# wedevxer/CUDA-AcceleratedVectorDatabaseEngine

Hardware: AMD Instinct MI355X
Metric: QPS + p99 latency, 10M×768D IVF-Flat k=10 nprobe=32, 1/2/4/8 MI355X (higher is better)
Workload: dtype fp32; 1 GPU; 10M x 768D IVF-Flat L2, nlist 4096, nprobe 32, batch 64, k 10; nvec=10000000, dim=768, nlist=4096, nprobe=32, batch=64, k=10, train_vectors=100000, parallelism=single GPU; 3 batches in flight

## Files before the change

cuda-acceleratedvectordatabaseengine_amd/csrc/engine.cpp:

```cpp
#include "engine.hpp"

#include <cmath>

#include "remove.hpp"
#include "remove_plan.hpp"

namespace vdbe {
thread_local std::string g_last_error;

namespace group {
void train_device(vdb_ivf* g, const float* d_v, uint64_t n);
void set_centroids(vdb_ivf* g, const float* c);
void add_host(vdb_ivf* g, const float* v, const uint64_t* ids, const uint32_t* lists, uint64_t n);
void add_device(vdb_ivf* g, const float* d_v, const uint64_t* d_ids, const uint32_t* d_lists, uint64_t n);
uint64_t gpu_bytes(const vdb_ivf* g, bool allocated);
void set_option(vdb_ivf* g, const std::string& name, int64_t value);
void synchronize(vdb_ivf* g);
uint64_t remove_ids(vdb_ivf* g, const std::vector<uint64_t>& sorted);
}

inline void no_group(const vdb_ivf* h, const char* what) {
    require(!h->is_group(), std::string(what) + " is not available on a group handle", VDB_ERR_UNSUPPORTED);
}
}

extern "C" {

const char* vdb_last_error(void) { return g_last_error.c_str(); }
const char* vdb_version(void) { return "vdb_ivf 0.1.0 (gfx950)"; }
#ifndef VDB_BUILD_ID
#define VDB_BUILD_ID "unknown"
#endif
const char* vdb_build_id(void) { return VDB_BUILD_ID; }

int vdb_device_count(int* count) {
    return guarded([&] {
        require(count != nullptr, "null count");
        HIPCHECK(hipGetDeviceCount(count));
    });
}

int vdb_ivf_create(const vdb_ivf_config* cfg, vdb_ivf** out) {
    return guarded([&] {
        require(cfg && out, "null argument");
        require(cfg->dimension > 0 && cfg->nlist > 0, "Invalid configuration: dimension and nlist must be > 0");
        require(cfg->metric >= 0 && cfg->metric <= 2, "unknown metric");
        require(cfg->nlist < (1u << 19) - 1, "nlist above 524286 is not supported", VDB_ERR_UNSUPPORTED);
        auto* h = new vdb_ivf();
        try {
            h->dim = cfg->dimension;
            h->nlist = cfg->nlist;
            h->d4 = (cfg->dimension + 4 * vdbk::kTileAlign - 1) / (4 * vdbk::kTileAlign) * vdbk::kTileAlign;
            h->dp = h->d4 * 4;
            h->metric = cfg->metric;
            h->device = cfg->device;
            h->max_gpu_memory = cfg->max_gpu_memory == ~0ull ? 0 : cfg->max_gpu_memory;
            h->set_device();
            HIPCHECK(hipStreamCreateWithFlags(&h->stream, hipStreamNonBlocking));
            for (auto& sl : h->slots) {
                HIPCHECK(hipStreamCreateWithFlags(&sl.side, hipStreamNonBlocking));
                HIPCHECK(hipEventCreateWithFlags(&sl.fork, hipEventDisableTiming));
                HIPCHECK(hipEventCreateWithFlags(&sl.join, hipEventDisableTiming));
                HIPCHECK(hipEventCreateWithFlags(&sl.done, hipEventDisableTiming));
            }
            h->cent_rm.ensure((size_t)h->nlist * h->dp);
            h->cent_il.ensure(cdiv(h->nlist, 64) * h->d4 * 64);
            HIPCHECK(hipMemsetAsync(h->cent_rm.p, 0, (size_t)h->nlist * h->dp * 4, h->stream));
            h->refresh_centroid_layout();
            h->count.assign(h->nlist, 0);
            h->owned.assign(h->nlist, 1);
            h->block_off.assign(h->nlist, 0);
            h->upload_directory();
        } catch (...) {
            delete h;
            throw;
        }
        *out = h;
    });
}

int vdb_ivf_destroy(vdb_ivf* h) {
    return guarded([&] {
        if (!h) return;
        (void)hipSetDevice(h->device);
        (void)hipStreamSynchronize(h->stream);
        delete h;
// ... 905 lines not shown
```

cuda-acceleratedvectordatabaseengine_amd/csrc/kernels.hpp:

```cpp
#pragma once
#include <hip/hip_runtime.h>
#include <stdint.h>

namespace vdbk {

constexpr int kMaxSegBlocks = 16;
constexpr int kTilePipe = 16;
constexpr uint32_t kMfmaBlockedRows = 1024;
#ifndef VDB_MERGE_BLOCKS
#define VDB_MERGE_BLOCKS 1024
#endif
constexpr uint32_t kMergeBlocks = VDB_MERGE_BLOCKS;
#ifndef VDB_TILE_PIPE_NARROW
#define VDB_TILE_PIPE_NARROW 4
#endif
constexpr int kTilePipeNarrow = VDB_TILE_PIPE_NARROW;
#ifndef VDB_SCAN_DIAG
#define VDB_SCAN_DIAG 0
#endif
constexpr int kTileAlign = kTilePipe;
constexpr int kMergeFan = 32;
constexpr int kWideGroup = 16;
constexpr int kWaveQueries = 16;
constexpr int kWideMinSeg = 4;
// ... 33 lines not shown
void launch_coarse_mfma(int metric, const float* cent_rm, uint32_t nlist, uint32_t dp, const float* qpad,
                        uint32_t B, float* approx, float* delta, hipStream_t s);
uint32_t rerank_rows(uint32_t dp, int regs);
void launch_select_rerank(int metric, int regs, const float* approx, const float* delta, const float* cent_rm,
                          uint32_t nlist, uint32_t dp, const float* qpad, uint32_t B, uint32_t P, uint32_t* cand,
                          uint32_t* probes, hipStream_t s);
void launch_assign_rerank(int metric, const float* approx, const float* delta, const float* cent_rm,
                          uint32_t nlist, uint32_t dp, const float* rows, uint32_t n, uint32_t* out, hipStream_t s);
void launch_select(int regs, const float* cd, uint32_t nlist, uint32_t B, uint32_t P, uint32_t* probes,
                   hipStream_t s);
void launch_plan(const uint32_t* probes, const uint32_t* nseg_local, const uint32_t* count_local,
                 uint32_t B, uint32_t P, uint32_t group, int wide, uint32_t segs_item, ScanItem* items, ScanItem* items_w,
                 uint32_t* counters, uint32_t* sorted_pair, uint32_t* part_base_sorted, uint32_t* part_base_qp,
                 uint32_t* nseg_qp, uint32_t* l1base_qp, uint2* l1_items, unsigned long long* stats,
                 uint32_t* thr, uint32_t mfma_min, hipStream_t s);
void launch_merge_partials(int regs, uint32_t grid_items, const uint32_t* probes, const uint32_t* count_global,
                           const uint32_t* nseg_qp, const uint32_t* part_base_qp, const uint32_t* l1base_qp,
                           const uint2* l1_items, const uint32_t* counters, const float* part_d,
                           const uint64_t* part_i, uint32_t k, float* l1_d, uint64_t* l1_i, hipStream_t s);
struct ScanArgs {
    const float4* __restrict__ arena;
    const uint64_t* __restrict__ ids;
    const uint64_t* __restrict__ block_off;
    const uint32_t* __restrict__ count;
    const float* __restrict__ qpad;
    const ScanItem* __restrict__ items;
    const ScanItem* __restrict__ items_w;
    const uint32_t* __restrict__ counters;
    const uint32_t* __restrict__ sorted_pair;
    const uint32_t* __restrict__ part_base_sorted;
    float* __restrict__ part_d;
    uint64_t* __restrict__ part_i;
    uint32_t d4;
    uint32_t k;
    uint32_t wide_stride;
    uint32_t* work;
    uint32_t seg_blocks;
    uint32_t segs_item;
    uint32_t fused;
    uint32_t* thr;
    uint32_t mfma_min;
    unsigned long long* mstats;
    const uint4* __restrict__ shadow = nullptr;
    const float* __restrict__ rows = nullptr;
    const float4* __restrict__ meta = nullptr;
    const uint16_t* __restrict__ qres = nullptr;
    const float4* __restrict__ pst = nullptr;
    const float* __restrict__ sscale = nullptr;
    const float* __restrict__ qscale = nullptr;
    uint32_t dp = 0;
    uint32_t P = 0;
    uint32_t wide_q = 16;
    uint32_t thr_every = 1;
    uint32_t* thr4 = nullptr;
    uint4* cand = nullptr;
    uint32_t cand_cap = 0;
    uint32_t* ccount = nullptr;
    uint32_t* ovf = nullptr;
    uint4* floor_out = nullptr;
    uint32_t floor_seq = 0;
    float* ublist = nullptr;
    uint32_t* ubcnt = nullptr;
    uint32_t rows_layout = 0;
    unsigned long long* stamps = nullptr;
    uint32_t stamps_cap = 0;
    uint32_t stamp_batch = 0;
};
size_t scan_wide_lds(uint32_t d4, uint32_t k, int waves);
bool scan_wide_fits(uint32_t d4, uint32_t k, int waves);
void launch_scan_narrow(int metric, int regs, uint32_t grid_blocks, const ScanArgs& a, hipStream_t s);
void launch_scan_wide(int metric, uint32_t grid_blocks, const ScanArgs& a, hipStream_t s, int waves = 4);
size_t scan_bounded_lds(uint32_t d4, uint32_t k);
bool scan_bounded_fits(uint32_t d4, uint32_t k);
void launch_scan_bounded(int metric, uint32_t grid_blocks, const ScanArgs& a, hipStream_t s);
bool scan_screen_fits(uint32_t k, uint32_t dp, uint32_t wq, bool deferred);
size_t screen_exact_lds(uint32_t d4);
void launch_gather_cache_rows(const float4* cache, uint32_t d4, const ulonglong2* src, uint32_t n, float* rows,
                              hipStream_t s);
size_t screen_shadow_u4(uint64_t blocks, uint32_t d4, bool i8 = false);
void launch_screen_build(const float4* arena, uint64_t blocks, uint32_t d4, const uint32_t* block_list,
                         const float* cent_rm, uint4* shadow, float* rows, float4* meta, hipStream_t s, float* sscale = nullptr);
void launch_screen_pairs(int metric, const float* q, uint32_t B, uint32_t P, const uint32_t* probes,
                         const float* cent_rm, uint32_t dp, uint16_t* qres, float4* pst, uint32_t* thr4, hipStream_t s,
                         uint32_t* scnt = nullptr, uint32_t* ovf = nullptr, uint32_t* counters = nullptr,
                         uint32_t* ubcnt = nullptr, float* qscale = nullptr);
void launch_scan_screen(int metric, uint32_t grid_blocks, const ScanArgs& a, hipStream_t s);
void launch_screen_collect(int metric, uint32_t grid_blocks, const ScanArgs& a, hipStream_t s);
void launch_screen_select(const ScanArgs& a, uint32_t BP, uint32_t* scnt, uint32_t* soff, uint2* surv,
                          const uint32_t* ovf, hipStream_t s, float* slb = nullptr);
void launch_screen_recheck(int metric, const ScanArgs& a, uint32_t BP, const uint32_t* probes, uint32_t* nseg_qp,
                           const uint32_t* soff, const uint32_t* scnt, const uint2* surv, const uint32_t* ovf,
                           const float* fetched, float* sdist, uint32_t max_surv, uint32_t smax, hipStream_t s,
                           const float* slb = nullptr);
void launch_tier_recheck(int phase, int metric, const ScanArgs& a, uint32_t BP, uint32_t* nseg_qp, const uint32_t* soff,
                         const uint32_t* scnt, const uint2* surv, const float* slb, uint8_t* mark, const uint32_t* rowmap,
                         const float* fetched, float* sdist, hipStream_t s);
void launch_slot_merge(int regs, const uint32_t* probes, const uint32_t* count_global,
                       const uint32_t* nseg_qp, const uint32_t* part_base_qp, const uint32_t* l1base_qp,
                       const float* part_d, const uint64_t* part_i, const float* l1_d, const uint64_t* l1_i,
                       uint32_t BP, uint32_t k, float* slot_d, uint64_t* slot_i, hipStream_t s);
void launch_query_merge(int regs, const uint32_t* probes, const uint32_t* count_global, const float* slot_d,
                        const uint64_t* slot_i, const float* carry_d, const uint64_t* carry_i,
                        uint32_t B, uint32_t P, uint32_t k, int stale, const uint32_t* req_start, uint32_t b0,
                        float* out_d, uint64_t* out_i, hipStream_t s);
void launch_carry(const uint32_t* probes, const uint32_t* count_global, uint32_t B, uint32_t P, uint32_t k,
                  const float* slot_d, const uint64_t* slot_i, const uint32_t* req_start, uint32_t b0,
                  float* carry_d, uint64_t* carry_i, hipStream_t s);
void launch_merge_fused(int regs, const uint32_t* probes, const uint32_t* count_global, const uint32_t* nseg_qp,
                        const uint32_t* part_base_qp, const float* part_d, const uint64_t* part_i, uint32_t B,
                        uint32_t P, uint32_t k, int stale, const uint32_t* req_start, uint32_t b0, const float* carry_d,
                        const uint64_t* carry_i, float* slot_d, uint64_t* slot_i, float* carry_nd, uint64_t* carry_ni,
                        float* out_d, uint64_t* out_i, hipStream_t s);
void launch_rank_merge(int regs, const float* d, const uint64_t* i, uint64_t d_stride, uint64_t i_stride,
                       uint32_t nranks, uint32_t n, uint32_t k, float* out_d, uint64_t* out_i, hipStream_t s);
void launch_fill_empty(uint64_t n, float* d, uint64_t* i, hipStream_t s);

void launch_interleave(const float* rows, uint64_t n, uint32_t dp, float4* blocks, hipStream_t s);
void launch_scatter_rows(const float* rows, const uint64_t* row_ids, const uint32_t* order, uint64_t n,
                         uint32_t dp, const uint64_t* dest_slot, float4* arena, uint64_t* arena_ids,
                         hipStream_t s);
void launch_copy_lists(const float4* old_arena, const uint64_t* old_ids, const uint64_t* old_off,
                       const uint64_t* new_off, const uint32_t* nblocks, uint32_t nlist, uint32_t d4,
                       float4* new_arena, uint64_t* new_ids, hipStream_t s);
void launch_export_list(const float4* arena, const uint64_t* ids, uint64_t block_off, uint32_t count,
                        uint32_t dim, uint32_t d4, float* out, uint64_t* out_ids, hipStream_t s);
void launch_assign(int metric, const float* vpad, uint64_t n, uint32_t dp, const float4* cent_il,
                   uint32_t nlist, uint32_t* out, hipStream_t s);
void launch_histogram(const uint32_t* keys, uint64_t n, uint32_t* counts, hipStream_t s);
void launch_mindist_init(float* mind, uint64_t n, hipStream_t s);
void launch_mindist_update(const float4* v_il, uint64_t n, uint32_t d4, const float* centroid_row,
                           float* mind, hipStream_t s);
void launch_centroid_update(const float* vpad, uint32_t dp, const uint32_t* order, const uint32_t* offsets,
                            const uint32_t* counts, uint32_t nlist, uint32_t dim, float* cent_rm,
                            hipStream_t s);
void launch_iota(uint32_t* out, uint64_t n, hipStream_t s);
void launch_slots_from_order(const uint32_t* sorted_keys, uint64_t n, const uint64_t* group_start,
                             const uint64_t* list_base_slot, uint64_t* dest_slot, hipStream_t s);
void launch_gen_normal(float* out, uint64_t n, uint64_t seed, uint64_t offset, hipStream_t s);
void launch_gen_mixture(float* out, uint64_t rows, uint32_t dim, const float* centers, uint32_t ncomp, float sigma,
                        uint64_t seed, uint64_t row0, hipStream_t s);
// ... 7 lines not shown
```

cuda-acceleratedvectordatabaseengine_amd/csrc/screen.hip:

```cpp
#pragma clang fp contract(off)

#include <hip/hip_runtime.h>

#include <algorithm>
#include <stdexcept>
#include <cfloat>
#include <type_traits>

#include "kernels.hpp"
#include "scan_common.hpp"
#include "wave_topk.hpp"

namespace vdbk {

typedef __bf16 bf16x8 __attribute__((ext_vector_type(8)));
typedef float f32x4 __attribute__((ext_vector_type(4)));
typedef uint32_t u32x4 __attribute__((ext_vector_type(4)));
typedef int i32x4 __attribute__((ext_vector_type(4)));

constexpr float kScreenHuge = 1125899906842624.0f;
constexpr int kRing = 512;
#ifndef VDB_SCREEN_EXACT_PIPE
#define VDB_SCREEN_EXACT_PIPE 4
#endif
constexpr int kExactPipe = VDB_SCREEN_EXACT_PIPE;
#ifndef VDB_SCREEN_EXACT_PIPE_END
#define VDB_SCREEN_EXACT_PIPE_END 8
#endif
constexpr int kExactPipeEnd = VDB_SCREEN_EXACT_PIPE_END;
#ifndef VDB_SCREEN_DIAG
#define VDB_SCREEN_DIAG 0
#endif

__device__ __forceinline__ uint32_t bf16_bits(float f) {
    const uint32_t b = __float_as_uint(f);
    const uint32_t ex = b & 0x7F800000u;
    if (ex == 0) return 0u;
    if (ex == 0x7F800000u) return 0x7FC0u;
    return (b + 0x7FFFu + ((b >> 16) & 1u)) >> 16;
}
__device__ __forceinline__ float bf16_val(uint32_t h) { return __uint_as_float(h << 16); }

__device__ __forceinline__ uint4 pack_bf16x8(const float4 lo, const float4 hi) {
    uint4 r;
    r.x = bf16_bits(lo.x) | (bf16_bits(lo.y) << 16);
    r.y = bf16_bits(lo.z) | (bf16_bits(lo.w) << 16);
    r.z = bf16_bits(hi.x) | (bf16_bits(hi.y) << 16);
    r.w = bf16_bits(hi.z) | (bf16_bits(hi.w) << 16);
    return r;
}

__device__ __forceinline__ float4 resid(const float4 x, const float4 c) {
    return make_float4((float)((double)x.x - c.x), (float)((double)x.y - c.y), (float)((double)x.z - c.z),
                       (float)((double)x.w - c.w));
}

__device__ __forceinline__ float ru(double v) { return __double2float_ru(v * (1.0 + 0x1p-30)); }
// ... 594 lines not shown
        if ((wv & 1) == 0 && (wv == 0 || split)) screen_partials(a, it, q0, nqh, seg0, it_d + ko, it_i + ko, true);
    }
    if (a.fused) drain_narrow();
}


__device__ __forceinline__ void block_sort64(float (&u)[4]) {
    const int l = lane_id() & 15;
    bitonic64_step<2, 1>(u, l);
    bitonic64_step<4, 2>(u, l), bitonic64_step<4, 1>(u, l);
    bitonic64_step<8, 4>(u, l), bitonic64_step<8, 2>(u, l), bitonic64_step<8, 1>(u, l);
    bitonic64_step<16, 8>(u, l), bitonic64_step<16, 4>(u, l), bitonic64_step<16, 2>(u, l), bitonic64_step<16, 1>(u, l);
    bitonic64_step<32, 16>(u, l), bitonic64_step<32, 8>(u, l), bitonic64_step<32, 4>(u, l);
    bitonic64_step<32, 2>(u, l), bitonic64_step<32, 1>(u, l);
    bitonic64_step<64, 32>(u, l), bitonic64_step<64, 16>(u, l), bitonic64_step<64, 8>(u, l);
    bitonic64_step<64, 4>(u, l), bitonic64_step<64, 2>(u, l), bitonic64_step<64, 1>(u, l);
}
__device__ __forceinline__ void merge_sorted64(float (&rl)[4], const float (&u)[4]) {
    const int l = lane_id() & 15;
#pragma unroll
    for (int v = 0; v < 4; ++v) {
        const float rv = __uint_as_float((uint32_t)__builtin_amdgcn_mov_dpp((int)__float_as_uint(u[3 - v]), 0x140, 0xF,
                                                                            0xF, false));
        rl[v] = fminf(rl[v], rv);
    }
    bitonic64_step<64, 32>(rl, l), bitonic64_step<64, 16>(rl, l), bitonic64_step<64, 8>(rl, l);
    bitonic64_step<64, 4>(rl, l), bitonic64_step<64, 2>(rl, l), bitonic64_step<64, 1>(rl, l);
}
__device__ __forceinline__ float row_elem(const float (&u)[4], int e) {
    const int v = e & 3;
    const float x = v == 0 ? u[0] : v == 1 ? u[1] : v == 2 ? u[2] : u[3];
    return __shfl(x, (lane_id() & ~15) + (e >> 2));
}

struct CandChunk {
    uint32_t base = 0, left = 0;
    uint32_t next = 0;
    uint32_t real = 0;
    bool pending = false;
};
__device__ __forceinline__ void pad_cand(const ScanArgs& a, uint32_t base, uint32_t n) {
    for (uint32_t i = (uint32_t)lane_id(); i < n; i += 64)
        if (base + i < a.cand_cap) a.cand[base + i] = make_uint4(~0u, 0u, 0u, ~0u);
}
__device__ __forceinline__ void finish_cand(const ScanArgs& a, CandChunk& cc) {
    pad_cand(a, cc.base, cc.left);
    if (cc.pending) pad_cand(a, cc.next, kCandChunk);
    if (cc.real && lane_id() == 0) atomicAdd(a.ccount + (kCtrReal - kCtrCand), cc.real);
    cc.left = 0;
    cc.real = 0;
    cc.pending = false;
}

template <int M, int KD, int NG, bool I8, bool W2>
__device__ __forceinline__ void collect_segment(const ScanArgs& a, const ScanItem it, const int q0, const int nq,
                                                const uint32_t seg, float4* rl_lds, uint32_t* s_thr,
                                                const float4* s_pst, const float* s_qsc, float4* s_mt, float* s_vs,
                                                const uint32_t residue, CandChunk& cc) {
    const int lane = lane_id();
    const uint32_t dp = a.dp, ks = dp >> (I8 ? 6 : 5);
    const uint32_t count = a.count[it.list];
    const uint32_t seg_vectors = a.seg_blocks * 64;
    const uint64_t b0 = a.block_off[it.list] + (uint64_t)seg * a.seg_blocks;
    const uint32_t v0 = seg * seg_vectors;
    const uint32_t nv = min(count - v0, seg_vectors);
    const uint32_t nb = (nv + 63) >> 6;
    const int k = (int)a.k, kq = ((int)a.k + 3) / 4;
    const uint32_t* pairs = a.sorted_pair + it.pair_start + q0;
    const float cm = (float)(4 * dp + 16) * 0x1.02p-24f;
    const float cr = (float)(dp + 2) * 0x1.02p-24f;
    const float cu = 0x1.02p-23f;
    auto pair_of = [&](int g) -> uint32_t {
        const uint32_t pr = pairs[g];
        return (pr >> 16) * a.P + (pr & 0xFFFFu);
    };
    const uint4* qa_row[NG];
#pragma unroll
    for (int gg = 0; gg < NG; ++gg)
        qa_row[gg] = (const uint4*)((const char*)a.qres + (size_t)pair_of(min(16 * gg + (lane & 15), nq - 1)) * dp *
                                                              (I8 ? 1 : 2)) +
                     (lane >> 4);
    uint32_t collected = 0;
    float gthr[NG][4], gq4[NG][4];
#pragma unroll
    for (int gg = 0; gg < NG; ++gg)
#pragma unroll
        for (int r = 0; r < 4; ++r) gthr[gg][r] = gq4[gg][r] = __builtin_inff();
    const uint32_t thr_every = W2 ? a.thr_every : 1u;
    const uint32_t spl = it.pair_start + q0 + min(lane & (16 * NG - 1), nq - 1);

    const uint4* sp = a.shadow + b0 * (uint64_t)ks * 256 + lane;
    uint4 xa[KD][4], qa[NG][KD];
#pragma unroll
    for (int u = 0; u < KD; ++u) {
#pragma unroll
        for (int vt = 0; vt < 4; ++vt) xa[u][vt] = ld_nt_u4(sp + (size_t)(u * 4 + vt) * 64);
#pragma unroll
        for (int gg = 0; gg < NG; ++gg) qa[gg][u] = qa_row[gg][4 * (u % ks)];
    }
    using AccT = std::conditional_t<I8, i32x4, f32x4>;
    for (uint32_t j = 0; j < nb; ++j) {
        const uint64_t mslot = (b0 + j) * 64 + lane;
        const float4 mt_l = a.meta[mslot];
        float vs_l = 0.0f;
        if constexpr (I8) vs_l = a.sscale[mslot];
        const bool thr_now = j % thr_every == 0;
        uint32_t gt_l = 0u;
        uint4 t4_l = make_uint4(0u, 0u, 0u, 0u);
        if (thr_now) {
            gt_l = a.thr[spl];
            t4_l = *(const uint4*)(a.thr4 + (size_t)spl * 4);
        }
        const bool reserve = !cc.pending && cc.left < kCandChunk / 2;
        uint32_t reply = 0;
        if (reserve && lane == 0) reply = atomicAdd(a.ccount, kCandChunk);
        AccT acc[NG][4];
#pragma unroll
        for (int gg = 0; gg < NG; ++gg)
#pragma unroll
            for (int vt = 0; vt < 4; ++vt) acc[gg][vt] = AccT{0, 0, 0, 0};
        for (uint32_t s0 = 0; s0 < ks; s0 += KD) {
            static_for<0, KD>([&](auto uu) {
                constexpr int u = decltype(uu)::value;
#pragma unroll
                for (int gg = 0; gg < NG; ++gg) {
                    if constexpr (I8) {
                        const i32x4 A = as_i32x4(qa[gg][u]);
#pragma unroll
                        for (int vt = 0; vt < 4; ++vt)
                            acc[gg][vt] =
                                __builtin_amdgcn_mfma_i32_16x16x64_i8(A, as_i32x4(xa[u][vt]), acc[gg][vt], 0, 0, 0);
                    } else {
                        const bf16x8 A = as_bf16x8(qa[gg][u]);
#pragma unroll
                        for (int vt = 0; vt < 4; ++vt)
                            acc[gg][vt] =
                                __builtin_amdgcn_mfma_f32_16x16x32_bf16(A, as_bf16x8(xa[u][vt]), acc[gg][vt], 0, 0, 0);
                    }
                }
                const uint64_t nxt = (uint64_t)j * ks + s0 + u + KD;
#pragma unroll
                for (int vt = 0; vt < 4; ++vt) xa[u][vt] = ld_nt_u4(sp + (nxt * 4 + vt) * 64);
#pragma unroll
                for (int gg = 0; gg < NG; ++gg) qa[gg][u] = qa_row[gg][4 * ((s0 + u + KD) % ks)];
            });
        }
        s_mt[lane] = mt_l;
        if constexpr (I8) s_vs[lane] = vs_l;
        if (reserve) {
            cc.next = __builtin_amdgcn_readfirstlane(reply);
            cc.pending = true;
        }
        float gthr_l = 0.0f, gq4_l = 0.0f;
        if (thr_now) {
            const float th4 =
                fmaxf(fmaxf(ord_dec(t4_l.x), ord_dec(t4_l.y)), fmaxf(ord_dec(t4_l.z), ord_dec(t4_l.w)));
            gthr_l = fminf(ord_dec(gt_l), th4);
            gq4_l = ord_dec(residue == 0 ? t4_l.x : residue == 1 ? t4_l.y : residue == 2 ? t4_l.z : t4_l.w);
        }
        __builtin_amdgcn_fence(__ATOMIC_RELEASE, "wavefront");
#pragma unroll
        for (int gg = 0; gg < NG; ++gg) {
            const int g0 = 16 * gg;
            float ubv[4][4];
            float4 pst[4];
            float qsc[4];
#pragma unroll
            for (int r = 0; r < 4; ++r) {
                const int gc = min(g0 + 4 * (lane >> 4) + r, nq - 1);
                pst[r] = s_pst[gc];
                if constexpr (I8) qsc[r] = s_qsc[gc];
            }
#pragma unroll
            for (int vt = 0; vt < 4; ++vt) {
                const float4 mt = s_mt[16 * vt + (lane & 15)];
                float vsc = 0.0f;
                if constexpr (I8) vsc = s_vs[16 * vt + (lane & 15)];
                const bool valid = j * 64 + 16 * vt + (lane & 15) < nv;
#pragma unroll
                for (int r = 0; r < 4; ++r) {
                    float dot;
                    if constexpr (I8) dot = (float)acc[gg][vt][r] * (qsc[r] * vsc);
                    else dot = acc[gg][vt][r];
                    const float4 ps = pst[r];
                    const float approx = M == kL2 ? (ps.x + mt.x) - 2.0f * dot : -(ps.x + dot);
                    const float an = ps.y + ps.z, bn = mt.y + mt.z;
                    const float cs = an * mt.z + ps.z * bn + ps.z * mt.z;
                    float del;
                    if (M == kL2) {
                        const float rest = 2.0f * (cs + cm * (an * bn)) + cu * (ps.x + mt.x + fabsf(approx));
                        del = rest + cr * (fabsf(approx) + rest);
                    } else {
                        del = cs + cm * (an * bn) + cr * (ps.y * mt.w) + cu * (ps.y * ps.w + an * bn + fabsf(approx));
                    }
                    del = del * 1.001f + 1e-30f;
                    const float ub = approx + del;
                    if constexpr (I8) acc[gg][vt][r] = __float_as_int(approx - del);
// ... 119 lines not shown
    }
    if (a.mstats && lane == 0) {
        atomicAdd(&a.mstats[0], (unsigned long long)collected);
        atomicAdd(&a.mstats[1], (unsigned long long)nb);
    }
}

__device__ __forceinline__ void overflow_item(const ScanArgs& a, uint32_t pair_start, uint32_t npairs, uint32_t t0,
                                              uint32_t nt) {
    for (uint32_t t = t0; t < npairs; t += nt) a.ovf[pair_start + t] = 1u;
    if (t0 == 0) a.ccount[kCtrOvf - kCtrCand] = 1u;
}

__device__ __forceinline__ void reset_rl(float4* rl_lds, int rows) {
    const int lane = lane_id();
    const float inf = __builtin_inff();
    for (int r = 0; r < rows; ++r) rl_lds[r * 64 + lane] = make_float4(inf, inf, inf, inf);
}

__device__ __forceinline__ void contribute_rl(const ScanArgs& a, const ScanItem it, const int q0, const int nq,
                                              const float4* rl_lds) {
    const int lane = lane_id();
    const int k = (int)a.k;
    for (int r = 0; r < (nq + 15) / 16 * 4; ++r) {
        const int g = 16 * (r >> 2) + 4 * (lane >> 4) + (r & 3);
        const uint32_t spi = it.pair_start + q0 + min(g, nq - 1);
        uint32_t slot = 0;
        if ((lane & 15) == 0 && g < nq) slot = atomicAdd(&a.ubcnt[spi], 1u);
        slot = __shfl(slot, lane & ~15);
        const float4 rv = rl_lds[r * 64 + lane];
        const float rl[4] = {rv.x, rv.y, rv.z, rv.w};
        if (g < nq && slot < (uint32_t)kUbLists) {
            float* dst = a.ublist + ((size_t)spi * kUbLists + slot) * k;
#pragma unroll
            for (int v = 0; v < 4; ++v) {
                const int e = 4 * (lane & 15) + v;
                if (e < k) dst[e] = rl[v];
            }
        }
    }
}

__device__ __forceinline__ void put_stamp(const ScanArgs& a, uint64_t w0, uint64_t t0, uint64_t w3) {
    const uint32_t i = atomicAdd((unsigned int*)a.stamps, 1u);
    if (i < a.stamps_cap) {
        unsigned long long* r = a.stamps + 2 + (size_t)i * 4;
        r[0] = ((uint64_t)a.stamp_batch << 40) | w0;
        r[1] = t0;
        r[2] = wall_clock64();
        r[3] = w3;
    }
}

template <int M, int KD, bool W2, bool I8>
__global__ __launch_bounds__(256, W2 ? 1 : 2) void ivf_screen_collect(ScanArgs a) {
    __shared__ uint32_t s_next, s_seg;
    __shared__ uint32_t s_thr[32];
    __shared__ uint32_t s_thr_w[4][16];
    __shared__ float4 s_rl[4][8 * 64];
    __shared__ float4 s_pst[32], s_pst_w[4][16];
    __shared__ float s_qsc[32], s_qsc_w[4][16];
    __shared__ float4 s_mt[4][64];
    __shared__ float s_vs[4][64];
    const uint32_t wv = wave_index();
    const int lane = lane_id();
    float4* rl = s_rl[wv];
    CandChunk cc;
    auto pair_stats = [&](uint32_t ps, uint32_t t, float4* dp4, float* dsc) {
        const uint32_t pr = a.sorted_pair[ps + t];
        const uint32_t pi = (pr >> 16) * a.P + (pr & 0xFFFFu);
        dp4[t] = a.pst[pi];
        if (I8) dsc[t] = a.qscale[pi];
    };

    auto drain_narrow = [&]() {
        const uint32_t n_narrow = a.counters[0];
        for (;;) {
            uint32_t idx = 0;
            if (lane == 0) idx = atomicAdd(&a.work[0], 1u);
            idx = __builtin_amdgcn_readfirstlane(idx);
            if (idx >= n_narrow) break;
            ScanItem it = a.items[idx];
            it.list = __builtin_amdgcn_readfirstlane(it.list);
            it.seg = __builtin_amdgcn_readfirstlane(it.seg);
            it.pair_start = __builtin_amdgcn_readfirstlane(it.pair_start);
            it.npairs = __builtin_amdgcn_readfirstlane(it.npairs);
            if (it.npairs > 16u) {
                overflow_item(a, it.pair_start, it.npairs, (uint32_t)lane, 64u);
                continue;
            }
            if (lane < (int)it.npairs) {
                s_thr_w[wv][lane] = a.thr[it.pair_start + lane];
                pair_stats(it.pair_start, lane, s_pst_w[wv], s_qsc_w[wv]);
            }
            __builtin_amdgcn_fence(__ATOMIC_RELEASE, "wavefront");
            const uint64_t t0 = a.stamps ? wall_clock64() : 0;
            reset_rl(rl, 4);
            collect_segment<M, KD, 1, I8, W2>(a, it, 0, (int)it.npairs, it.seg, rl, s_thr_w[wv], s_pst_w[wv],
                                              s_qsc_w[wv], s_mt[wv], s_vs[wv], it.seg & 3u, cc);
            contribute_rl(a, it, 0, (int)it.npairs, rl);
            if (a.stamps && lane == 0)
                put_stamp(a, ((uint64_t)idx << 16) | blockIdx.x, t0, it.npairs | (1u << 8) | (1u << 16) | ((uint64_t)it.list << 32));
        }
    };

    const uint32_t n_wide = a.counters[3];
    if (a.stamps && threadIdx.x == 0) put_stamp(a, blockIdx.x, wall_clock64(), 2u << 16);
    if (a.fused && blockIdx.x + a.fused >= gridDim.x) drain_narrow();
    for (;;) {
        if (threadIdx.x == 0) s_next = atomicAdd(&a.work[1], 1u);
        __syncthreads();
        const uint32_t b = s_next;
        if (b >= n_wide) break;
        const uint64_t t_item = a.stamps ? wall_clock64() : 0;
        ScanItem it = a.items_w[b];
        it.list = __builtin_amdgcn_readfirstlane(it.list);
        it.seg = __builtin_amdgcn_readfirstlane(it.seg);
        it.pair_start = __builtin_amdgcn_readfirstlane(it.pair_start);
        it.npairs = __builtin_amdgcn_readfirstlane(it.npairs);
        const int nq = (int)it.npairs;
        if (nq > (W2 ? 32 : 16)) {
            overflow_item(a, it.pair_start, (uint32_t)nq, threadIdx.x, blockDim.x);
            __syncthreads();
            continue;
        }
        if (threadIdx.x == 0) s_seg = 0;
        if (threadIdx.x < (uint32_t)nq) {
            s_thr[threadIdx.x] = a.thr[it.pair_start + threadIdx.x];
            pair_stats(it.pair_start, threadIdx.x, s_pst, s_qsc);
        }
        __syncthreads();
        const uint32_t seg_vectors = a.seg_blocks * 64;
        const uint32_t nseg = (a.count[it.list] + seg_vectors - 1) / seg_vectors;
        const uint32_t seg0 = it.seg * a.segs_item, seg1 = min(nseg, seg0 + a.segs_item);
        reset_rl(rl, nq > 16 ? 8 : 4);
        bool any = false;
        for (;;) {
            uint32_t sg = 0;
            if (lane == 0) sg = atomicAdd(&s_seg, 1u);
            sg = seg0 + __builtin_amdgcn_readfirstlane(sg);
            if (sg >= seg1) break;
            if (W2 && nq > 16)
                collect_segment<M, KD, 2, I8, W2>(a, it, 0, nq, sg, rl, s_thr, s_pst, s_qsc, s_mt[wv], s_vs[wv], wv, cc);
            else
                collect_segment<M, KD, 1, I8, W2>(a, it, 0, nq, sg, rl, s_thr, s_pst, s_qsc, s_mt[wv], s_vs[wv], wv, cc);
            any = true;
        }
        if (any) contribute_rl(a, it, 0, nq, rl);
        __syncthreads();
        if (a.stamps && threadIdx.x == 0)
            put_stamp(a, ((uint64_t)b << 16) | blockIdx.x, t_item, (uint32_t)nq | ((seg1 - seg0) << 8) | ((uint64_t)it.list << 32));
    }
    if (a.fused) drain_narrow();
    finish_cand(a, cc);
}

bool scan_screen_fits(uint32_t k, uint32_t dp, uint32_t wq, bool deferred) {
    return k >= 1 && k <= 64 && dp % 64 == 0 && (wq == 16 || wq == 32) && screen_exact_lds(dp / 4) <= kLdsBytes / 2 &&
           (deferred || screen_item_lds(k, wq) + 4 * screen_wave_lds(k) + 256 <= kLdsBytes / 2);
}

size_t screen_shadow_u4(uint64_t blocks, uint32_t d4, bool i8) {
    return (size_t)(blocks + 2) * d4 * (i8 ? 16 : 32);
}

void launch_screen_build(const float4* arena, uint64_t blocks, uint32_t d4, const uint32_t* block_list,
                         const float* cent_rm, uint4* shadow, float* rows, float4* meta, hipStream_t s, float* sscale) {
    if (!blocks) return;
    const uint32_t g = (uint32_t)std::min<uint64_t>((blocks + 3) / 4, 8192);
    if (sscale) ivf_screen_build_i8<<<g, 256, 0, s>>>(arena, blocks, d4, block_list, cent_rm, shadow, rows, meta, sscale);
    else ivf_screen_build<<<g, 256, 0, s>>>(arena, blocks, d4, block_list, cent_rm, shadow, rows, meta);
}

void launch_screen_pairs(int metric, const float* q, uint32_t B, uint32_t P, const uint32_t* probes,
                         const float* cent_rm, uint32_t dp, uint16_t* qres, float4* pst, uint32_t* thr4, hipStream_t s,
                         uint32_t* scnt, uint32_t* ovf, uint32_t* counters, uint32_t* ubcnt, float* qscale) {
    const uint32_t BP = B * P;
    if (!BP) return;
    const uint32_t g = std::min<uint32_t>((BP + 3) / 4, 2048);
    if (qscale) {
        if (metric == kL2)
            ivf_screen_pairs_i8<kL2><<<g, 256, 0, s>>>(q, BP, P, probes, cent_rm, dp, (int8_t*)qres, qscale, pst, thr4,
                                                       scnt, ovf, counters, ubcnt);
        else
            ivf_screen_pairs_i8<kIP><<<g, 256, 0, s>>>(q, BP, P, probes, cent_rm, dp, (int8_t*)qres, qscale, pst, thr4,
                                                       scnt, ovf, counters, ubcnt);
        return;
    }
    if (metric == kL2)
        ivf_screen_pairs<kL2><<<g, 256, 0, s>>>(q, BP, P, probes, cent_rm, dp, qres, pst, thr4, scnt, ovf, counters, ubcnt);
    else
        ivf_screen_pairs<kIP><<<g, 256, 0, s>>>(q, BP, P, probes, cent_rm, dp, qres, pst, thr4, scnt, ovf, counters, ubcnt);
}

#ifndef VDB_COLLECT_KD
#define VDB_COLLECT_KD 4
#endif
void launch_screen_collect(int metric, uint32_t grid_blocks, const ScanArgs& a, hipStream_t s) {
    if (!grid_blocks) return;
    if (a.wide_q != 16 && a.wide_q != 32) throw std::length_error("launch_screen_collect: items of 16 or 32 queries only");
    const bool w2 = a.wide_q > 16;
    const uint32_t g = std::min<uint32_t>(grid_blocks, w2 ? kPersistentBlocks / 2 : kPersistentBlocks);
    auto go = [&](auto m_c, auto w_c, auto i_c) {
        constexpr int Mm = decltype(m_c)::value;
        constexpr bool Ww = decltype(w_c)::value;
        constexpr bool Ii = decltype(i_c)::value;
        constexpr int KW = Ii ? 6 : 8;
        const uint32_t ks = a.dp / (Ii ? 64 : 32);
        if (Ww && ks % KW == 0) ivf_screen_collect<Mm, KW, Ww, Ii><<<g, 256, 0, s>>>(a);
        else if (!Ww && VDB_COLLECT_KD != 4 && ks % VDB_COLLECT_KD == 0)
            ivf_screen_collect<Mm, VDB_COLLECT_KD, Ww, Ii><<<g, 256, 0, s>>>(a);
        else if (ks % 4 == 0) ivf_screen_collect<Mm, 4, Ww, Ii><<<g, 256, 0, s>>>(a);
        else if (ks % 2 == 0) ivf_screen_collect<Mm, 2, Ww, Ii><<<g, 256, 0, s>>>(a);
        else ivf_screen_collect<Mm, 1, Ww, Ii><<<g, 256, 0, s>>>(a);
    };
    auto go_w = [&](auto m_c, auto i_c) {
        if (w2) go(m_c, std::true_type{}, i_c);
        else go(m_c, std::false_type{}, i_c);
    };
    auto go_i = [&](auto m_c) {
        if (a.sscale) go_w(m_c, std::true_type{});
        else go_w(m_c, std::false_type{});
    };
    if (metric == kL2) go_i(std::integral_constant<int, kL2>{});
    else go_i(std::integral_constant<int, kIP>{});
}

void launch_scan_screen(int metric, uint32_t grid_blocks, const ScanArgs& a, hipStream_t s) {
    if (!grid_blocks) return;
    static const bool raised = [] {
        const void* f[] = {(const void*)ivf_scan_screen<kL2, 4>, (const void*)ivf_scan_screen<kL2, 2>,
                           (const void*)ivf_scan_screen<kIP, 4>, (const void*)ivf_scan_screen<kIP, 2>};
        for (const void* fn : f)
            (void)hipFuncSetAttribute(fn, hipFuncAttributeMaxDynamicSharedMemorySize, (int)(kLdsBytes / 2 - 256));
        (void)hipGetLastError();
        return true;
    }();
    (void)raised;
    const uint32_t g = std::min<uint32_t>(grid_blocks, kPersistentBlocks);
    const size_t lds = screen_item_lds(a.k, a.wide_q) + 4 * screen_wave_lds(a.k);
    const bool kd4 = (a.dp / 32) % 4 == 0;
    if (metric == kL2) {
        if (kd4) ivf_scan_screen<kL2, 4><<<g, 256, lds, s>>>(a);
        else ivf_scan_screen<kL2, 2><<<g, 256, lds, s>>>(a);
    } else {
        if (kd4) ivf_scan_screen<kIP, 4><<<g, 256, lds, s>>>(a);
        else ivf_scan_screen<kIP, 2><<<g, 256, lds, s>>>(a);
    }
}

}
```

include/vdb_ivf.h:

```cpp
#ifndef VDB_IVF_H
#define VDB_IVF_H

#include <stddef.h>
#include <stdint.h>

#ifdef __cplusplus
extern "C" {
#endif

enum {
    VDB_OK = 0,
    VDB_ERR_INVALID_ARGUMENT = -1,
    VDB_ERR_DEVICE = -2,
    VDB_ERR_OUT_OF_MEMORY = -3,
    VDB_ERR_UNSUPPORTED = -4,
    VDB_ERR_STATE = -5
};

enum { VDB_METRIC_L2 = 0, VDB_METRIC_INNER_PRODUCT = 1, VDB_METRIC_COSINE = 2 };

typedef struct vdb_ivf vdb_ivf;

typedef struct vdb_ivf_config {
    uint32_t dimension;
    uint32_t nlist;
    int32_t metric;
    int32_t use_gpu;
    uint64_t max_gpu_memory;
    int32_t device;
} vdb_ivf_config;

typedef struct vdb_ivf_profile {
    uint64_t batches;
    uint64_t scan_launches;
    double scan_ms;
    double coarse_ms;
    double total_ms;
    uint64_t scan_vectors;
    uint64_t distinct_lists;
    uint64_t work_items;
    uint64_t scan_bytes;
    uint64_t pair_vectors;
    uint64_t exact_reranks;
    uint64_t bounded_blocks;
    uint64_t computed_vectors;
    double local_merge_ms;
    uint64_t exchanges;
    double exchange_ms;
    double rank_merge_ms;
    uint64_t screen_collected;
    double collect_ms;
    double recheck_ms;
    uint64_t screen_floor_batches;
    uint64_t screen_floor_trips;
    uint32_t screen_shadow;
    uint32_t reserved0;
} vdb_ivf_profile;

const char* vdb_last_error(void);
const char* vdb_version(void);
const char* vdb_build_id(void);
int vdb_device_count(int* count);

int vdb_ivf_create(const vdb_ivf_config* config, vdb_ivf** out);
int vdb_ivf_destroy(vdb_ivf* index);

int vdb_ivf_train(vdb_ivf* index, const float* vectors, uint64_t n);
int vdb_ivf_train_device(vdb_ivf* index, const float* d_vectors, uint64_t n);
int vdb_ivf_set_centroids(vdb_ivf* index, const float* centroids);
int vdb_ivf_get_centroids(vdb_ivf* index, float* centroids);

int vdb_ivf_add(vdb_ivf* index, const float* vectors, const uint64_t* ids, uint64_t n);
int vdb_ivf_add_device(vdb_ivf* index, const float* d_vectors, const uint64_t* d_ids, uint64_t n);

int vdb_ivf_add_to_lists(vdb_ivf* index, const float* vectors, const uint64_t* ids, const uint32_t* lists,
                         uint64_t n);
int vdb_ivf_assign_device(vdb_ivf* index, const float* d_vectors, uint64_t n, uint32_t* d_lists);
int vdb_ivf_add_to_lists_device(vdb_ivf* index, const float* d_vectors, const uint64_t* d_ids,
                                const uint32_t* d_lists, uint64_t n);
int vdb_ivf_remove_ids(vdb_ivf* index, const uint64_t* ids, uint64_t n, uint64_t* removed);
int vdb_remove_last_timing(double* mark_ms, double* plan_ms, double* compact_ms, uint64_t* rows_kept);
int vdb_ivf_save(vdb_ivf* index, const char* path);
int vdb_ivf_load(vdb_ivf* index, const char* path);

int vdb_ivf_search(vdb_ivf* index, const float* queries, uint32_t n, uint32_t nprobe, uint32_t k,
                   float* distances, uint64_t* ids);
int vdb_ivf_search_device(vdb_ivf* index, const float* d_queries, uint32_t n, uint32_t nprobe,
                          uint32_t k, float* d_distances, uint64_t* d_ids, void* stream);

int vdb_ivf_set_shard(vdb_ivf* index, uint32_t rank, uint32_t world);
int vdb_ivf_plan_shard(vdb_ivf* index, uint32_t rank, uint32_t world, const uint64_t* final_sizes);
int vdb_merge_ranks_device(const float* d_dist, const uint64_t* d_ids, uint32_t nranks, uint32_t n,
                           uint32_t k, float* d_out_dist, uint64_t* d_out_ids, void* stream);
uint64_t vdb_rank_record_bytes(uint32_t n, uint32_t k);
int vdb_merge_ranks_packed_device(const void* d_records, uint32_t nranks, uint32_t n, uint32_t k,
                                  float* d_out_dist, uint64_t* d_out_ids, void* stream);
int vdb_shard_plan(const uint64_t* list_sizes, uint32_t nlist, uint32_t world, uint32_t* owner);
int vdb_shard_plan_probe_weighted(const uint64_t* list_sizes, const uint64_t* probe_counts, uint64_t n_sample,
                                  uint32_t batch, uint32_t nlist, uint32_t world, uint32_t* owner);
int vdb_ivf_probe_census(vdb_ivf* index, const float* d_rows, uint64_t n, uint32_t nprobe, uint64_t* counts);
int vdb_ivf_set_shard_owners(vdb_ivf* index, uint32_t rank, uint32_t world, const uint32_t* owner);
int vdb_ivf_plan_shard_owners(vdb_ivf* index, uint32_t rank, uint32_t world, const uint64_t* final_sizes,
                              const uint32_t* owner);

#define VDB_COMM_ID_BYTES 128
int vdb_comm_unique_id(void* id);
int vdb_ivf_attach_comm(vdb_ivf* index, const void* id, uint32_t rank, uint32_t world);
int vdb_ivf_detach_comm(vdb_ivf* index);
int vdb_ivf_comm_status(vdb_ivf* index, uint64_t* exchanges_issued, uint64_t* exchanges_done);
int vdb_ivf_create_group(const vdb_ivf_config* config, const int* devices, uint32_t ndevices, vdb_ivf** out);
uint32_t vdb_ivf_group_size(const vdb_ivf* index);
int vdb_ivf_list_owners(vdb_ivf* index, uint32_t* owner);

int vdb_ivf_warmup(vdb_ivf* index, const uint32_t* lists, uint32_t n);
// ... 61 lines not shown
```

Baseline: 48430 queries/s.

## Stage quantized query rows in LDS for screen-collect kernel

Adds a dynamic-LDS staging path in the screen collect kernel: quantized query residue rows for an item are copied once into padded shared memory and read from there inside the MFMA loop, instead of being held in registers or re-read from global memory for every k-step. This is meant to cut global/L2 traffic and register pressure for the query operand. It also clamps the shadow prefetch index so the pipeline does not read past the last block. Items whose staged rows would not fit fall back to the overflow path. The launch raises the kernel's max dynamic LDS size once per device, and a mode query is exported through the C API.

```diff
diff --git a/cuda-acceleratedvectordatabaseengine_amd/csrc/engine.cpp b/cuda-acceleratedvectordatabaseengine_amd/csrc/engine.cpp
--- a/cuda-acceleratedvectordatabaseengine_amd/csrc/engine.cpp
+++ b/cuda-acceleratedvectordatabaseengine_amd/csrc/engine.cpp
@@ -32,6 +32,9 @@
 #define VDB_BUILD_ID "unknown"
 #endif
 const char* vdb_build_id(void) { return VDB_BUILD_ID; }
+int vdb_collect_stage_mode(uint32_t dp, int i8, uint32_t wide_q) {
+    return vdbk::collect_stage_mode(dp, i8 != 0, wide_q);
+}
 
 int vdb_device_count(int* count) {
     return guarded([&] {
diff --git a/cuda-acceleratedvectordatabaseengine_amd/csrc/kernels.hpp b/cuda-acceleratedvectordatabaseengine_amd/csrc/kernels.hpp
--- a/cuda-acceleratedvectordatabaseengine_amd/csrc/kernels.hpp
+++ b/cuda-acceleratedvectordatabaseengine_amd/csrc/kernels.hpp
@@ -109,6 +109,7 @@
     uint32_t P = 0;
     uint32_t wide_q = 16;
     uint32_t thr_every = 1;
+    uint32_t stage_bytes = 0;
     uint32_t* thr4 = nullptr;
     uint4* cand = nullptr;
     uint32_t cand_cap = 0;
@@ -143,6 +144,8 @@
                          uint32_t* ubcnt = nullptr, float* qscale = nullptr);
 void launch_scan_screen(int metric, uint32_t grid_blocks, const ScanArgs& a, hipStream_t s);
 void launch_screen_collect(int metric, uint32_t grid_blocks, const ScanArgs& a, hipStream_t s);
+int collect_stage_mode(uint32_t dp, bool i8, uint32_t wq);
+size_t collect_stage_lds(uint32_t dp, bool i8, uint32_t wq);
 void launch_screen_select(const ScanArgs& a, uint32_t BP, uint32_t* scnt, uint32_t* soff, uint2* surv,
                           const uint32_t* ovf, hipStream_t s, float* slb = nullptr);
 void launch_screen_recheck(int metric, const ScanArgs& a, uint32_t BP, const uint32_t* probes, uint32_t* nseg_qp,
diff --git a/cuda-acceleratedvectordatabaseengine_amd/csrc/screen.hip b/cuda-acceleratedvectordatabaseengine_amd/csrc/screen.hip
--- a/cuda-acceleratedvectordatabaseengine_amd/csrc/screen.hip
+++ b/cuda-acceleratedvectordatabaseengine_amd/csrc/screen.hip
@@ -3,6 +3,7 @@
 #include <hip/hip_runtime.h>
 
 #include <algorithm>
+#include <atomic>
 #include <stdexcept>
 #include <cfloat>
 #include <type_traits>
@@ -703,11 +704,19 @@
     cc.pending = false;
 }
 
-template <int M, int KD, int NG, bool I8, bool W2>
+#ifndef VDB_COLLECT_STAGE
+#define VDB_COLLECT_STAGE 1
+#endif
+#ifndef VDB_COLLECT_CLAMP
+#define VDB_COLLECT_CLAMP 1
+#endif
+
+template <int M, int KD, int NG, bool I8, bool W2, bool STG>
 __device__ __forceinline__ void collect_segment(const ScanArgs& a, const ScanItem it, const int q0, const int nq,
                                                 const uint32_t seg, float4* rl_lds, uint32_t* s_thr,
                                                 const float4* s_pst, const float* s_qsc, float4* s_mt, float* s_vs,
-                                                const uint32_t residue, CandChunk& cc) {
+                                                const uint32_t residue, CandChunk& cc, const uint4* s_qa,
+                                                const uint32_t stride4) {
     const int lane = lane_id();
     const uint32_t dp = a.dp, ks = dp >> (I8 ? 6 : 5);
     const uint32_t count = a.count[it.list];
@@ -727,10 +736,11 @@
     };
     const uint4* qa_row[NG];
 #pragma unroll
-    for (int gg = 0; gg < NG; ++gg)
-        qa_row[gg] = (const uint4*)((const char*)a.qres + (size_t)pair_of(min(16 * gg + (lane & 15), nq - 1)) * dp *
-                                                              (I8 ? 1 : 2)) +
-                     (lane >> 4);
+    for (int gg = 0; gg < NG; ++gg) {
+        const int g = min(16 * gg + (lane & 15), nq - 1);
+        if constexpr (STG) qa_row[gg] = s_qa + (uint32_t)g * stride4 + (lane >> 4);
+        else qa_row[gg] = (const uint4*)((const char*)a.qres + (size_t)pair_of(g) * dp * (I8 ? 1 : 2)) + (lane >> 4);
+    }
     uint32_t collected = 0;
     float gthr[NG][4], gq4[NG][4];
 #pragma unroll
@@ -741,13 +751,17 @@
     const uint32_t spl = it.pair_start + q0 + min(lane & (16 * NG - 1), nq - 1);
 
     const uint4* sp = a.shadow + b0 * (uint64_t)ks * 256 + lane;
-    uint4 xa[KD][4], qa[NG][KD];
+    const uint64_t ks_last = VDB_COLLECT_CLAMP && !W2 && nb ? (uint64_t)nb * ks - 1 : ~0ull;
+    uint4 xa[KD][4], qa[NG][STG ? 1 : KD];
 #pragma unroll
     for (int u = 0; u < KD; ++u) {
-#pragma unroll
-        for (int vt = 0; vt < 4; ++vt) xa[u][vt] = ld_nt_u4(sp + (size_t)(u * 4 + vt) * 64);
-#pragma unroll
-        for (int gg = 0; gg < NG; ++gg) qa[gg][u] = qa_row[gg][4 * (u % ks)];
+        const uint64_t nxt = (uint64_t)u < ks_last ? (uint64_t)u : ks_last;
+#pragma unroll
+        for (int vt = 0; vt < 4; ++vt) xa[u][vt] = ld_nt_u4(sp + (nxt * 4 + vt) * 64);
+        if constexpr (!STG) {
+#pragma unroll
+            for (int gg = 0; gg < NG; ++gg) qa[gg][u] = qa_row[gg][4 * (u % ks)];
+        }
     }
     using AccT = std::conditional_t<I8, i32x4, f32x4>;
     for (uint32_t j = 0; j < nb; ++j) {
@@ -775,25 +789,30 @@
                 constexpr int u = decltype(uu)::value;
 #pragma unroll
                 for (int gg = 0; gg < NG; ++gg) {
+                    uint4 av;
+                    if constexpr (STG) av = qa_row[gg][4 * (s0 + u)];
+                    else av = qa[gg][u];
                     if constexpr (I8) {
-                        const i32x4 A = as_i32x4(qa[gg][u]);
+                        const i32x4 A = as_i32x4(av);
 #pragma unroll
                         for (int vt = 0; vt < 4; ++vt)
                             acc[gg][vt] =
                                 __builtin_amdgcn_mfma_i32_16x16x64_i8(A, as_i32x4(xa[u][vt]), acc[gg][vt], 0, 0, 0);
                     } else {
-                        const bf16x8 A = as_bf16x8(qa[gg][u]);
+                        const bf16x8 A = as_bf16x8(av);
 #pragma unroll
                         for (int vt = 0; vt < 4; ++vt)
                             acc[gg][vt] =
                                 __builtin_amdgcn_mfma_f32_16x16x32_bf16(A, as_bf16x8(xa[u][vt]), acc[gg][vt], 0, 0, 0);
                     }
                 }
-                const uint64_t nxt = (uint64_t)j * ks + s0 + u + KD;
+                const uint64_t nx = (uint64_t)j * ks + s0 + u + KD, nxt = nx < ks_last ? nx : ks_last;
 #pragma unroll
                 for (int vt = 0; vt < 4; ++vt) xa[u][vt] = ld_nt_u4(sp + (nxt * 4 + vt) * 64);
-#pragma unroll
-                for (int gg = 0; gg < NG; ++gg) qa[gg][u] = qa_row[gg][4 * ((s0 + u + KD) % ks)];
+                if constexpr (!STG) {
+#pragma unroll
+                    for (int gg = 0; gg < NG; ++gg) qa[gg][u] = qa_row[gg][4 * ((s0 + u + KD) % ks)];
+                }
             });
         }
         s_mt[lane] = mt_l;
@@ -1019,19 +1038,44 @@
     }
 }
 
-template <int M, int KD, bool W2, bool I8>
+template <bool W2>
+struct CollectLds {
+    float4 rl[4][(W2 ? 8 : 4) * 64];
+    float4 pst[32], pst_w[4][16];
+    float4 mt[4][64];
+    float vs[4][64];
+    float qsc[32], qsc_w[4][16];
+    uint32_t thr[32];
+    uint32_t thr_w[4][16];
+    uint32_t next, seg;
+};
+
+constexpr uint32_t kStagePad = 16;
+template <bool I8>
+__device__ __forceinline__ void stage_rows(const ScanArgs& a, uint32_t pair_start, uint32_t nq, uint4* dst,
+                                           uint32_t stride4, uint32_t t0, uint32_t nt) {
+    const uint32_t r4 = a.dp * (I8 ? 1u : 2u) / 16u;
+    const uint4* src = (const uint4*)a.qres;
+    for (uint32_t e = t0; e < nq * r4; e += nt) {
+        const uint32_t g = e / r4, c = e - g * r4;
+        const uint32_t pr = a.sorted_pair[pair_start + g];
+        dst[g * stride4 + c] = src[(size_t)((pr >> 16) * a.P + (pr & 0xFFFFu)) * r4 + c];
+    }
+}
+
+template <int M, int KD, bool W2, bool I8, int STG>
 __global__ __launch_bounds__(256, W2 ? 1 : 2) void ivf_screen_collect(ScanArgs a) {
-    __shared__ uint32_t s_next, s_seg;
-    __shared__ uint32_t s_thr[32];
-    __shared__ uint32_t s_thr_w[4][16];
-    __shared__ float4 s_rl[4][8 * 64];
-    __shared__ float4 s_pst[32], s_pst_w[4][16];
-    __shared__ float s_qsc[32], s_qsc_w[4][16];
-    __shared__ float4 s_mt[4][64];
-    __shared__ float s_vs[4][64];
+    __shared__ CollectLds<W2> L;
+    extern __shared__ uint4 s_stage[];
+    uint32_t& s_next = L.next;
+    uint32_t& s_seg = L.seg;
+    uint32_t* const s_thr = L.thr;
+    float4* const s_pst = L.pst;
+    float* const s_qsc = L.qsc;
     const uint32_t wv = wave_index();
     const int lane = lane_id();
-    float4* rl = s_rl[wv];
+    float4* rl = L.rl[wv];
+    const uint32_t stride4 = (a.dp * (I8 ? 1u : 2u) + kStagePad) / 16u;
     CandChunk cc;
     auto pair_stats = [&](uint32_t ps, uint32_t t, float4* dp4, float* dsc) {
         const uint32_t pr = a.sorted_pair[ps + t];
@@ -1052,19 +1096,21 @@
             it.seg = __builtin_amdgcn_readfirstlane(it.seg);
             it.pair_start = __builtin_amdgcn_readfirstlane(it.pair_start);
             it.npairs = __builtin_amdgcn_readfirstlane(it.npairs);
-            if (it.npairs > 16u) {
+            if (it.npairs > 16u || (STG == 2 && (16u * wv + it.npairs) * stride4 * 16u > a.stage_bytes)) {
                 overflow_item(a, it.pair_start, it.npairs, (uint32_t)lane, 64u);
                 continue;
             }
             if (lane < (int)it.npairs) {
-                s_thr_w[wv][lane] = a.thr[it.pair_start + lane];
-                pair_stats(it.pair_start, lane, s_pst_w[wv], s_qsc_w[wv]);
-            }
+                L.thr_w[wv][lane] = a.thr[it.pair_start + lane];
+                pair_stats(it.pair_start, lane, L.pst_w[wv], L.qsc_w[wv]);
+            }
+            uint4* qa_w = s_stage + 16u * wv * stride4;
+            if constexpr (STG == 2) stage_rows<I8>(a, it.pair_start, it.npairs, qa_w, stride4, (uint32_t)lane, 64u);
             __builtin_amdgcn_fence(__ATOMIC_RELEASE, "wavefront");
             const uint64_t t0 = a.stamps ? wall_clock64() : 0;
             reset_rl(rl, 4);
-            collect_segment<M, KD, 1, I8, W2>(a, it, 0, (int)it.npairs, it.seg, rl, s_thr_w[wv], s_pst_w[wv],
-                                              s_qsc_w[wv], s_mt[wv], s_vs[wv], it.seg & 3u, cc);
+            collect_segment<M, KD, 1, I8, W2, STG == 2>(a, it, 0, (int)it.npairs, it.seg, rl, L.thr_w[wv], L.pst_w[wv],
+                                                        L.qsc_w[wv], L.mt[wv], L.vs[wv], it.seg & 3u, cc, qa_w, stride4);
             contribute_rl(a, it, 0, (int)it.npairs, rl);
             if (a.stamps && lane == 0)
                 put_stamp(a, ((uint64_t)idx << 16) | blockIdx.x, t0, it.npairs | (1u << 8) | (1u << 16) | ((uint64_t)it.list << 32));
@@ -1086,7 +1132,7 @@
         it.pair_start = __builtin_amdgcn_readfirstlane(it.pair_start);
         it.npairs = __builtin_amdgcn_readfirstlane(it.npairs);
         const int nq = (int)it.npairs;
-        if (nq > (W2 ? 32 : 16)) {
+        if (nq > (W2 ? 32 : 16) || (STG > 0 && (uint32_t)nq * stride4 * 16u > a.stage_bytes)) {
             overflow_item(a, it.pair_start, (uint32_t)nq, threadIdx.x, blockDim.x);
             __syncthreads();
             continue;
@@ -1096,6 +1142,7 @@
             s_thr[threadIdx.x] = a.thr[it.pair_start + threadIdx.x];
             pair_stats(it.pair_start, threadIdx.x, s_pst, s_qsc);
         }
+        if constexpr (STG > 0) stage_rows<I8>(a, it.pair_start, (uint32_t)nq, s_stage, stride4, threadIdx.x, blockDim.x);
         __syncthreads();
         const uint32_t seg_vectors = a.seg_blocks * 64;
         const uint32_t nseg = (a.count[it.list] + seg_vectors - 1) / seg_vectors;
@@ -1108,9 +1155,11 @@
             sg = seg0 + __builtin_amdgcn_readfirstlane(sg);
             if (sg >= seg1) break;
             if (W2 && nq > 16)
-                collect_segment<M, KD, 2, I8, W2>(a, it, 0, nq, sg, rl, s_thr, s_pst, s_qsc, s_mt[wv], s_vs[wv], wv, cc);
+                collect_segment<M, KD, 2, I8, W2, (STG > 0)>(a, it, 0, nq, sg, rl, s_thr, s_pst, s_qsc, L.mt[wv], L.vs[wv],
+                                                             wv, cc, s_stage, stride4);
             else
-                collect_segment<M, KD, 1, I8, W2>(a, it, 0, nq, sg, rl, s_thr, s_pst, s_qsc, s_mt[wv], s_vs[wv], wv, cc);
+                collect_segment<M, KD, 1, I8, W2, (STG > 0)>(a, it, 0, nq, sg, rl, s_thr, s_pst, s_qsc, L.mt[wv], L.vs[wv],
+                                                             wv, cc, s_stage, stride4);
             any = true;
         }
         if (any) contribute_rl(a, it, 0, nq, rl);
@@ -1160,30 +1209,74 @@
         ivf_screen_pairs<kIP><<<g, 256, 0, s>>>(q, BP, P, probes, cent_rm, dp, qres, pst, thr4, scnt, ovf, counters, ubcnt);
 }
 
+static size_t collect_stage_budget(bool w2) {
+    return w2 ? kLdsBytes - sizeof(CollectLds<true>) : kLdsBytes / 2 - sizeof(CollectLds<false>);
+}
+int collect_stage_mode(uint32_t dp, bool i8, uint32_t wq) {
+    if (!VDB_COLLECT_STAGE || wq > 16) return 0;
+    const size_t row = (size_t)dp * (i8 ? 1 : 2) + kStagePad, budget = collect_stage_budget(wq > 16);
+    return 64 * row <= budget ? 2 : (wq > 16 ? 32 : 16) * row <= budget ? 1 : 0;
+}
+size_t collect_stage_lds(uint32_t dp, bool i8, uint32_t wq) {
+    const int mode = collect_stage_mode(dp, i8, wq);
+    return ((size_t)dp * (i8 ? 1 : 2) + kStagePad) * (mode == 2 ? 64 : mode == 1 ? (wq > 16 ? 32 : 16) : 0);
+}
+
+template <int M, int KD, bool W2, bool I8, int STG>
+static void run_screen_collect(uint32_t g, const ScanArgs& a, hipStream_t s) {
+    if constexpr (STG > 0) {
+        static std::atomic<uint64_t> raised{0};
+        int dev = 0;
+        (void)hipGetDevice(&dev);
+        const uint64_t bit = 1ull << (dev & 63);
+        if (!(raised.load(std::memory_order_relaxed) & bit)) {
+            (void)hipFuncSetAttribute((const void*)ivf_screen_collect<M, KD, W2, I8, STG>,
+                                      hipFuncAttributeMaxDynamicSharedMemorySize, (int)collect_stage_budget(W2));
+            (void)hipGetLastError();
+            raised.fetch_or(bit, std::memory_order_relaxed);
+        }
+    }
+    ivf_screen_collect<M, KD, W2, I8, STG><<<g, 256, a.stage_bytes, s>>>(a);
+}
+
 #ifndef VDB_COLLECT_KD
 #define VDB_COLLECT_KD 4
 #endif
-void launch_screen_collect(int metric, uint32_t grid_blocks, const ScanArgs& a, hipStream_t s) {
+void launch_screen_collect(int metric, uint32_t grid_blocks, const ScanArgs& args, hipStream_t s) {
     if (!grid_blocks) return;
-    if (a.wide_q != 16 && a.wide_q != 32) throw std::length_error("launch_screen_collect: items of 16 or 32 queries only");
+    if (args.wide_q != 16 && args.wide_q != 32)
+        throw std::length_error("launch_screen_collect: items of 16 or 32 queries only");
+    ScanArgs a = args;
+    const int stage = collect_stage_mode(a.dp, a.sscale != nullptr, a.wide_q);
+    a.stage_bytes = (uint32_t)collect_stage_lds(a.dp, a.sscale != nullptr, a.wide_q);
     const bool w2 = a.wide_q > 16;
     const uint32_t g = std::min<uint32_t>(grid_blocks, w2 ? kPersistentBlocks / 2 : kPersistentBlocks);
-    auto go = [&](auto m_c, auto w_c, auto i_c) {
+    auto go = [&](auto m_c, auto w_c, auto i_c, auto s_c) {
         constexpr int Mm = decltype(m_c)::value;
         constexpr bool Ww = decltype(w_c)::value;
         constexpr bool Ii = decltype(i_c)::value;
+        constexpr int Ss = decltype(s_c)::value;
         constexpr int KW = Ii ? 6 : 8;
         const uint32_t ks = a.dp / (Ii ? 64 : 32);
-        if (Ww && ks % KW == 0) ivf_screen_collect<Mm, KW, Ww, Ii><<<g, 256, 0, s>>>(a);
+        if (Ww && ks % KW == 0) run_screen_collect<Mm, KW, Ww, Ii, Ss>(g, a, s);
         else if (!Ww && VDB_COLLECT_KD != 4 && ks % VDB_COLLECT_KD == 0)
-            ivf_screen_collect<Mm, VDB_COLLECT_KD, Ww, Ii><<<g, 256, 0, s>>>(a);
-        else if (ks % 4 == 0) ivf_screen_collect<Mm, 4, Ww, Ii><<<g, 256, 0, s>>>(a);
-        else if (ks % 2 == 0) ivf_screen_collect<Mm, 2, Ww, Ii><<<g, 256, 0, s>>>(a);
-        else ivf_screen_collect<Mm, 1, Ww, Ii><<<g, 256, 0, s>>>(a);
+            run_screen_collect<Mm, VDB_COLLECT_KD, Ww, Ii, Ss>(g, a, s);
+        else if (ks % 4 == 0) run_screen_collect<Mm, 4, Ww, Ii, Ss>(g, a, s);
+        else if (ks % 2 == 0) run_screen_collect<Mm, 2, Ww, Ii, Ss>(g, a, s);
+        else run_screen_collect<Mm, 1, Ww, Ii, Ss>(g, a, s);
+    };
+    auto go_s = [&](auto m_c, auto w_c, auto i_c) {
+        if constexpr (decltype(w_c)::value) {
+            go(m_c, w_c, i_c, std::integral_constant<int, 0>{});
+        } else {
+            if (stage == 2) go(m_c, w_c, i_c, std::integral_constant<int, 2>{});
+            else if (stage == 1) go(m_c, w_c, i_c, std::integral_constant<int, 1>{});
+            else go(m_c, w_c, i_c, std::integral_constant<int, 0>{});
+        }
     };
     auto go_w = [&](auto m_c, auto i_c) {
-        if (w2) go(m_c, std::true_type{}, i_c);
-        else go(m_c, std::false_type{}, i_c);
+        if (w2) go_s(m_c, std::true_type{}, i_c);
+        else go_s(m_c, std::false_type{}, i_c);
     };
     auto go_i = [&](auto m_c) {
         if (a.sscale) go_w(m_c, std::true_type{});
diff --git a/include/vdb_ivf.h b/include/vdb_ivf.h
--- a/include/vdb_ivf.h
+++ b/include/vdb_ivf.h
@@ -60,6 +60,7 @@
 const char* vdb_last_error(void);
 const char* vdb_version(void);
 const char* vdb_build_id(void);
+int vdb_collect_stage_mode(uint32_t dp, int i8, uint32_t wide_q);
 int vdb_device_count(int* count);
 
 int vdb_ivf_create(const vdb_ivf_config* config, vdb_ivf** out);
```

Result: no change. 48750 queries/s (median of 2 runs) (+0.7%).
